# yzhang511/multi_modal_foundation_model

Measured on AMD Instinct MI355X. Metric: pretrain samples/sec (T=100 bins/modality, d_model=256, 5+5 layers, spike+behaviour masked pretraining step), higher is better.
Workload: dtype bf16; 1 GPU; BASELINE.json configs[1]: 1 session, ap(668 neurons)+behaviour(2), d_model=256, heads=8, mlp=512, 5 enc + 5 dec layers, T=100 (L=200 tokens), dropout 0.4/0.2, AdamW+OneCycleLR, mixed objectives; per_gpu_batch=1024, global_batch=1024, seq_len=200, parallelism=dp1

## Files before the change

include/mmfm.h:

```cpp
#ifndef MMFM_H
#define MMFM_H
#include <stdint.h>
#ifdef __cplusplus
extern "C" {
#endif

#define MMFM_VERSION 401
#define MMFM_F32 0
#define MMFM_BF16 1
#define MMFM_MLP_GELU 0
#define MMFM_MLP_RELU 1
#define MMFM_MLP_SIGMOID 2
#define MMFM_MLP_GELU_TANH 3

typedef void* mmfm_stream;

typedef struct {
    const void* state;
    uint32_t site;
    float p;
} mmfm_dropout;

int mmfm_version(void);
const char* mmfm_last_error(void);
// ... 134 lines not shown
    float* bp;
    int N, K;
    int tile0;
    int scalar_gain;
    void* WpP;
    void* WpTP;
} mmfm_prep_entry;
int mmfm_prep_weights(const mmfm_prep_entry* entries, int n_entries, int total_tiles, mmfm_stream stream);

typedef struct {
    int64_t R;
    int K, N;
    const void* x; int ldx;
    const void* w; int ldw;
    const float* bias;
    int ln; float eps;
    void* xhat; float* rstd;
    const void* residual; int ldr;
    void* y; int ldy;
    int stream_out;
    int rotate;
    int ln_bwd;
    const void* bwd_xhat; const float* bwd_rstd;
} mmfm_rowgemm_desc;
int mmfm_rowgemm(const mmfm_rowgemm_desc* d, mmfm_stream stream);

typedef struct {
    int64_t R;
    const void* x; int ldx;
    float eps;
    const void* w_up; const float* b_up;
    const void* w_down; const float* b_down;
    mmfm_dropout drop;
    void* y; int ldy;
    void* xhat; float* rstd;
    const void* dy; int lddy;
    const void* w_down_t;
    const void* w_up_t;
    void* t1; void* g; void* du;
    void* dx; int lddx;
    int rotate;
    int scalenorm;
    int act;
    float act_beta;
} mmfm_mlp_desc;
int mmfm_mlp_fwd(const mmfm_mlp_desc* d, mmfm_stream stream);
// ... 14 lines not shown
```

multi_modal_foundation_model_amd/_lib.py:

```python
from __future__ import annotations

import ctypes as C
import os
import re

import torch

_HERE = os.path.dirname(os.path.abspath(__file__))
LIB_PATH = os.environ.get("MMFM_LIB") or os.path.join(_HERE, "libmmfm_hip.so")
HEADER_PATH = os.path.join(os.path.dirname(_HERE), "include", "mmfm.h")

F32, BF16 = 0, 1
ATTN_DIAG, ATTN_CAUSAL, ATTN_SEP = 1, 2, 4
ACT_NONE, ACT_GELU, ACT_SOFTSIGN, ACT_GELU_GRAD, ACT_SOFTSIGN_GRAD, ACT_SOFTSIGN_GRAD_OUT = 0, 1, 2, 3, 4, 5
ACT_RELU, ACT_RELU_GRAD, ACT_SIGMOID, ACT_SIGMOID_GRAD, ACT_GELU_TANH, ACT_GELU_TANH_GRAD = 6, 7, 8, 9, 10, 11
MLP_GELU, MLP_RELU, MLP_SIGMOID, MLP_GELU_TANH = 0, 1, 2, 3


class MmfmError(RuntimeError):
    pass


class Dropout(C.Structure):
    _fields_ = [("state", C.c_void_p), ("site", C.c_uint32), ("p", C.c_float)]
# ... 15 lines not shown
    _fields_ = [("dtype", C.c_int), ("B", C.c_int), ("heads", C.c_int), ("Lq", C.c_int), ("Lk", C.c_int), ("dh", C.c_int),
                ("q", C.c_void_p), ("k", C.c_void_p), ("v", C.c_void_p), ("ldq", C.c_int), ("ldk", C.c_int),
                ("ldv", C.c_int), ("o", C.c_void_p), ("ldo", C.c_int), ("lse", C.c_void_p), ("keypad", C.c_void_p),
                ("mod_id", C.c_void_p), ("flags", C.c_int), ("scale", C.c_float), ("drop_p", Dropout),
                ("drop_o", Dropout), ("d_o", C.c_void_p), ("lddo", C.c_int), ("dq", C.c_void_p), ("dk", C.c_void_p),
                ("dv", C.c_void_p), ("lddq", C.c_int), ("lddk", C.c_int), ("lddv", C.c_int), ("keepbits", C.c_void_p)]


class PrepEntry(C.Structure):
    _fields_ = [("W", C.c_void_p), ("gamma", C.c_void_p), ("beta", C.c_void_p), ("bias", C.c_void_p), ("Wp", C.c_void_p),
                ("WpT", C.c_void_p), ("bp", C.c_void_p), ("N", C.c_int), ("K", C.c_int), ("tile0", C.c_int), ("scalar_gain", C.c_int),
                ("WpP", C.c_void_p), ("WpTP", C.c_void_p)]


class ReduceEntry(C.Structure):
    _fields_ = [("dst", C.c_void_p), ("src", C.c_void_p), ("n", C.c_int64), ("slab_stride", C.c_int64), ("nslabs", C.c_int32),
                ("accumulate", C.c_int32), ("chunk0", C.c_int32), ("pad_", C.c_int32)]


class RowGemmDesc(C.Structure):
    _fields_ = [("R", C.c_int64), ("K", C.c_int), ("N", C.c_int), ("x", C.c_void_p), ("ldx", C.c_int), ("w", C.c_void_p),
                ("ldw", C.c_int), ("bias", C.c_void_p), ("ln", C.c_int), ("eps", C.c_float), ("xhat", C.c_void_p),
                ("rstd", C.c_void_p), ("residual", C.c_void_p), ("ldr", C.c_int), ("y", C.c_void_p), ("ldy", C.c_int),
                ("stream_out", C.c_int), ("rotate", C.c_int), ("ln_bwd", C.c_int), ("bwd_xhat", C.c_void_p), ("bwd_rstd", C.c_void_p)]


class MlpDesc(C.Structure):
    _fields_ = [("R", C.c_int64), ("x", C.c_void_p), ("ldx", C.c_int), ("eps", C.c_float), ("w_up", C.c_void_p),
                ("b_up", C.c_void_p), ("w_down", C.c_void_p), ("b_down", C.c_void_p), ("drop", Dropout), ("y", C.c_void_p),
                ("ldy", C.c_int), ("xhat", C.c_void_p), ("rstd", C.c_void_p), ("dy", C.c_void_p), ("lddy", C.c_int),
                ("w_down_t", C.c_void_p), ("w_up_t", C.c_void_p), ("t1", C.c_void_p), ("g", C.c_void_p), ("du", C.c_void_p),
                ("dx", C.c_void_p), ("lddx", C.c_int), ("rotate", C.c_int), ("scalenorm", C.c_int),
                ("act", C.c_int), ("act_beta", C.c_float)]


_vp, _i, _i64, _f = C.c_void_p, C.c_int, C.c_int64, C.c_float
_PROTOS = {
    "mmfm_version": (C.c_int, []),
    "mmfm_last_error": (C.c_char_p, []),
    "mmfm_device_check": (C.c_int, [_i]),
    "mmfm_rng_seed": (C.c_int, [_vp, C.c_uint64, _vp]),
    "mmfm_rng_advance": (C.c_int, [_vp, _vp]),
    "mmfm_gemm": (C.c_int, [C.POINTER(GemmDesc), _vp]),
    "mmfm_gemm_pair": (C.c_int, [_vp, _vp, _vp]),
    "mmfm_gemm_dw_tiles": (C.c_int, [_i, _i, _i]),
    "mmfm_reduce_slabs": (C.c_int, [_vp, _vp, _i64, _i, _i64, _i, _vp]),
    "mmfm_reduce_slabs_multi": (C.c_int, [_vp, _i, _i, _vp]),
# ... 66 lines not shown
```

multi_modal_foundation_model_amd/csrc/rowgemm.hip:

```cpp
#define MMFM_ACT_LOAD_AUX 2
#include "rowchain.h"
#include <stdlib.h>
#include <algorithm>
#include <type_traits>

using namespace rowchain;

namespace {

constexpr int NT = 256, NW = 4;

constexpr int BIAS_MAX = 1024;

template <int KP, int LN, bool NTS, int NWV>
__global__ __launch_bounds__(NWV * 64, (KP == 1 ? 2 : 1)) void rowgemm_kernel(const mmfm_rowgemm_desc d) {
    constexpr int NT = NWV * 64, NW = NWV;
    __shared__ __attribute__((aligned(16))) char smem[LDS_BYTES + NW * STG_BYTES + BIAS_MAX * 4];
    const int t = threadIdx.x, lane = t & 63, wave = __builtin_amdgcn_readfirstlane(t >> 6), m = lane & 31, h = lane >> 5;
    const int npair = d.N >> 6, cpp = 2 * npair * KP;
    const int64_t npass = (d.R + 32 * NW - 1) / (32 * NW);
    const int my_passes = blockIdx.x < npass ? (int)((npass - 1 - blockIdx.x) / gridDim.x) + 1 : 0;
    if (my_passes == 0) return;
    const uint16_t* W = reinterpret_cast<const uint16_t*>(d.w);
    const int ldw = d.ldw;
// ... 218 lines not shown
            f32x16 o[2];
#pragma unroll
            for (int j = 0; j < 2; ++j) {
                const f32x16 xt = unstage_tile(xstash + tp * STG_BYTES, j, m, h);
#pragma unroll
                for (int i = 0; i < 16; ++i) o[j][i] = rs * (acc[2 * tp + j][i] - s1 - xt[i] * s2);
            }
            stage_lines(stg, rl, lane);
#pragma unroll
            for (int j = 0; j < 2; ++j) {
                const f32x16 r = unstage_tile(stg, j, m, h);
#pragma unroll
                for (int i = 0; i < 16; ++i) o[j][i] += r[i];
            }
            stage_tile(stg, 0, m, h, o[0]);
            stage_tile(stg, 1, m, h, o[1]);
            flush_lines<false>(stg, Y, wrow0, ldyb, 128u * tp, lane);
        }
    }
}

#pragma clang diagnostic push
#pragma clang diagnostic ignored "-Winline-asm"
template <int KP, int NORM>
__global__ __launch_bounds__(NT) void rowgemm_lnbwd_a_kernel(const mmfm_rowgemm_desc d) {
    constexpr int RING_B = RINGA_SLOTS * CHUNK;
    extern __shared__ __attribute__((aligned(16))) char smem[];
    const int t = threadIdx.x, lane = t & 63, wave = __builtin_amdgcn_readfirstlane(t >> 6), m = lane & 31, h = lane >> 5;
    constexpr int cpp = 8 * KP;
    const int64_t npass = (d.R + 32 * NW - 1) / (32 * NW);
    const int my_passes = blockIdx.x < npass ? (int)((npass - 1 - blockIdx.x) / gridDim.x) + 1 : 0;
    if (my_passes == 0) return;
    const __amdgpu_buffer_rsrc_t rs_w = wbuf(d.w);
    const uint32_t ldwb = (uint32_t)d.ldw * 2u;
    auto src = [=](int g) {
        const int idx = g % cpp, tt = idx / KP, p = idx - tt * KP;
        AChunk c;
        c.rs = rs_w; c.off = (uint32_t)(32 * tt) * ldwb + 512u * (uint32_t)p; c.ldb = ldwb; c.kind = 0;
        return c;
    };
    char* stg = smem + RING_B + wave * STG_BYTES;
    char* xstash = smem + RING_B + NW * STG_BYTES + wave * 4 * STG_BYTES;
    const GBuf X = gbuf(d.x, d.R * d.ldx * 2), Y = gbuf(d.y, d.R * d.ldy * 2), RES = gbuf(d.residual, d.R * d.ldr * 2);
    const GBuf XH = gbuf(d.bwd_xhat, d.R * 512), RS = gbuf(d.bwd_rstd, d.R * 4);
    const uint32_t ldxb = d.ldx * 2, ldyb = d.ldy * 2, ldrb = d.ldr * 2;
    const ALane<NT> ring_al = alane_init<NT>(t, ldwb, 0u);
    const AFrag fr = afrag_init(m, h);
    RINGA_DECL(NT);
    RINGA_START((uint32_t)(uintptr_t)(__attribute__((address_space(3))) char*)smem, my_passes * cpp, src);
    for (int pi = 0; pi < my_passes; ++pi) {
        const uint32_t wrow0 = (uint32_t)(((int64_t)(blockIdx.x + (int64_t)pi * gridDim.x) * NW + wave) * 32);
        opnd x[16 * KP];
        {
            Lines xl[4];
#pragma unroll
            for (int tp = 0; tp < 4; ++tp) xl[tp] = fetch_lines(XH, wrow0, 512u, 128u * tp, lane);
            load_rows_lines<4 * KP>(stg, x, X, wrow0, ldxb, lane, m, h);
#pragma unroll
            for (int tp = 0; tp < 4; ++tp) stage_lines(xstash + tp * STG_BYTES, xl[tp], lane);
        }
        float rs = ld4f(RS, (wrow0 + m) * 4u);
        f32x16 acc[8];
#pragma unroll
        for (int tt = 0; tt < 8; ++tt) {
            acc[tt] = zero16();
#pragma unroll
            for (int p = 0; p < KP; ++p) {
                uint32_t slot;
                RINGA_SYNC(src, slot, 0);
                acc[tt] = mma16a<4>(slot, fr, x + 16 * p, acc[tt], [&](int g_) { RINGA_PIECE(g_); });
            }
        }
        float s1 = 0.f, s2 = 0.f;
#pragma unroll
        for (int tp = 0; tp < 4; ++tp) {
#pragma unroll
            for (int j = 0; j < 2; ++j) {
                const f32x16 xt = unstage_tile(xstash + tp * STG_BYTES, j, m, h);
#pragma unroll
                for (int i = 0; i < 16; ++i) { s1 += acc[2 * tp + j][i]; s2 = fmaf(acc[2 * tp + j][i], xt[i], s2); }
            }
        }
        s1 = xhalf(s1);
        s2 = xhalf(s2);
        norm_bwd_stats<NORM>(s1, s2, rs);
        Lines rl4[4];
#pragma unroll
        for (int tp = 0; tp < 4; ++tp) rl4[tp] = fetch_lines(RES, wrow0, ldrb, 128u * tp, lane);
#pragma unroll
        for (int tp = 0; tp < 4; ++tp) {
            const Lines& rl = rl4[tp];
            f32x16 o[2];
#pragma unroll
            for (int j = 0; j < 2; ++j) {
                const f32x16 xt = unstage_tile(xstash + tp * STG_BYTES, j, m, h);
#pragma unroll
                for (int i = 0; i < 16; ++i) o[j][i] = rs * (acc[2 * tp + j][i] - s1 - xt[i] * s2);
            }
            stage_lines(stg, rl, lane);
#pragma unroll
            for (int j = 0; j < 2; ++j) {
                const f32x16 r = unstage_tile(stg, j, m, h);
#pragma unroll
                for (int i = 0; i < 16; ++i) o[j][i] += r[i];
            }
            stage_tile(stg, 0, m, h, o[0]);
            stage_tile(stg, 1, m, h, o[1]);
            flush_lines<false>(stg, Y, wrow0, ldyb, 128u * tp, lane);
        }
    }
}
#pragma clang diagnostic pop

template <int KP, int NORM>
__global__ __launch_bounds__(512) void rowgemm_lnbwd8_kernel(const mmfm_rowgemm_desc d) {
    constexpr int NT = 512, NW = 8, NPAIR = 4;
    __shared__ __attribute__((aligned(16))) char smem[2 * CHUNK2 + NW * STG_BYTES + NW * 32 * 8];
    const int t = threadIdx.x, lane = t & 63, wave = __builtin_amdgcn_readfirstlane(t >> 6), m = lane & 31, h = lane >> 5;
    const int half = wave >> 2, pw = wave & 3;
    constexpr int cpp = 4 * KP;
    const int64_t npass = (d.R + 32 * NPAIR - 1) / (32 * NPAIR);
    const int my_passes = blockIdx.x < npass ? (int)((npass - 1 - blockIdx.x) / gridDim.x) + 1 : 0;
    if (my_passes == 0) return;
    const uint16_t* W = reinterpret_cast<const uint16_t*>(d.w);
    const int ldw = d.ldw;
    auto src = [=](int g) {
        const int idx = g % cpp, p = idx >> 2, j = idx & 3;
        WChunk2 c;
        c.s[0].base = W + (size_t)(32 * j) * ldw + 256 * p; c.s[0].ld = ldw; c.s[0].kind = 0;
        c.s[1].base = W + (size_t)(32 * (4 + j)) * ldw + 256 * p; c.s[1].ld = ldw; c.s[1].kind = 0;
        return c;
    };
    char* stg = smem + 2 * CHUNK2 + wave * STG_BYTES;
// ... 126 lines not shown
    return (int)std::max<int64_t>(1, std::min<int64_t>(npass, 256 * per_cu));
}

}

extern "C" int mmfm_rowgemm(const mmfm_rowgemm_desc* dp, mmfm_stream stream) {
    const mmfm_rowgemm_desc d = *dp;
    MMFM_REQUIRE(d.x && d.w && d.y && d.R > 0, "mmfm_rowgemm: null operand / empty problem");
    MMFM_REQUIRE(d.K == 256 || d.K == 512 || d.K == 768, "mmfm_rowgemm: K = %d (256, 512 or 768 only)", d.K);
    MMFM_REQUIRE(d.N > 0 && d.N % 64 == 0, "mmfm_rowgemm: N = %d must be a positive multiple of 64", d.N);
    MMFM_REQUIRE(d.ldx % 8 == 0 && d.ldw % 8 == 0 && d.ldy % 8 == 0 && d.ldx >= d.K && d.ldw >= d.K && d.ldy >= d.N,
                 "mmfm_rowgemm: leading dimensions (%d, %d, %d) must be multiples of 8 and cover the rows", d.ldx, d.ldw, d.ldy);
    auto al16 = [](const void* p) { return ((uintptr_t)p & 15) == 0; };
    MMFM_REQUIRE(al16(d.x) && al16(d.w) && al16(d.y) && al16(d.residual) && al16(d.xhat) && al16(d.bwd_xhat) && al16(d.bias),
                 "mmfm_rowgemm: operands must be 16-byte aligned");
    MMFM_REQUIRE(!d.residual || (d.ldr % 8 == 0 && d.ldr >= d.N), "mmfm_rowgemm: ldr %d", d.ldr);
    MMFM_REQUIRE(d.ln >= 0 && d.ln <= 2 && d.ln_bwd >= 0 && d.ln_bwd <= 2, "mmfm_rowgemm: ln = %d, ln_bwd = %d (0, 1 = LayerNorm, 2 = ScaleNorm)", d.ln, d.ln_bwd);
    MMFM_REQUIRE(!d.ln || d.K == 256, "mmfm_rowgemm: the norm prologue needs K = 256");
    const int64_t maxld = std::max<int64_t>(std::max(d.ldx, d.ldy), std::max(d.ldr, 256));
    MMFM_REQUIRE((d.R + 128) * maxld * 2 < (int64_t)1 << 31, "mmfm_rowgemm: tensors beyond 2 GiB are not addressable by the 32-bit buffer offsets");
    MMFM_REQUIRE(d.N <= BIAS_MAX, "mmfm_rowgemm: N = %d > %d", d.N, BIAS_MAX);
    static const int per_cu_env = [] { const char* e = getenv("MMFM_ROWGEMM_WG_PER_CU"); return e ? atoi(e) : 0; }();
    hipStream_t st = (hipStream_t)stream;
    if (d.ln_bwd) {
        MMFM_REQUIRE(d.N == 256 && d.bwd_xhat && d.bwd_rstd && !d.ln && !d.bias, "mmfm_rowgemm: ln_bwd needs N = 256, x_hat, rstd, no bias/ln");
        const bool sn = d.ln_bwd == 2;
        if (d.K == 256) {
            dim3 grid(grid_for(d.R, per_cu_env > 0 ? per_cu_env : 1, 4)), block(512);
            if (sn) hipLaunchKernelGGL((rowgemm_lnbwd8_kernel<1, 2>), grid, block, 0, st, d);
            else hipLaunchKernelGGL((rowgemm_lnbwd8_kernel<1, 1>), grid, block, 0, st, d);
        } else {
            dim3 grid(grid_for(d.R, per_cu_env > 0 ? per_cu_env : 1)), block(NT);
            static const int ring_env = [] { const char* e = getenv("MMFM_ROWGEMM_RING"); return (e ? atoi(e) : 3) & 2; }();
            constexpr int LDS_L = RINGA_SLOTS * CHUNK + NW * STG_BYTES + NW * 4 * STG_BYTES;
#define LNB_A(KP, NORM)                                                                                                     \
            {                                                                                                               \
                if (int rc = mmfm_lds_opt_in(reinterpret_cast<const void*>(rowgemm_lnbwd_a_kernel<KP, NORM>), LDS_L, "mmfm_rowgemm")) return rc; \
                hipLaunchKernelGGL((rowgemm_lnbwd_a_kernel<KP, NORM>), grid, block, LDS_L, st, d);                           \
            }
            if (ring_env && d.K == 512) { if (sn) LNB_A(2, 2) else LNB_A(2, 1) }
            else if (ring_env) { if (sn) LNB_A(3, 2) else LNB_A(3, 1) }
            else if (d.K == 512) { if (sn) hipLaunchKernelGGL((rowgemm_lnbwd_kernel<2, 2>), grid, block, 0, st, d); else hipLaunchKernelGGL((rowgemm_lnbwd_kernel<2, 1>), grid, block, 0, st, d); }
            else { if (sn) hipLaunchKernelGGL((rowgemm_lnbwd_kernel<3, 2>), grid, block, 0, st, d); else hipLaunchKernelGGL((rowgemm_lnbwd_kernel<3, 1>), grid, block, 0, st, d); }
#undef LNB_A
        }
    } else {
#define RG_LAUNCH(KP, LN)                                                                                   \
    if (d.stream_out) hipLaunchKernelGGL((rowgemm_kernel<KP, LN, true, 4>), grid, block, 0, st, d);         \
    else hipLaunchKernelGGL((rowgemm_kernel<KP, LN, false, 4>), grid, block, 0, st, d);
        if (d.K != 256) {
            dim3 grid(grid_for(d.R, per_cu_env > 0 ? per_cu_env : 1, 4)), block(256);
            if (d.K == 512) { RG_LAUNCH(2, 0) } else { RG_LAUNCH(3, 0) }
        } else {
            dim3 grid(grid_for(d.R, per_cu_env > 0 ? per_cu_env : 2, 4)), block(256);
            static const int ring_env = [] { const char* e = getenv("MMFM_ROWGEMM_RING"); return (e ? atoi(e) : 3) & 1; }();
            if (ring_env && (!d.residual || (d.N == 256 && !d.ln))) {
                constexpr int LDS_A = RINGA_SLOTS * CHUNK + 4 * STG_BYTES + BIAS_MAX * 4;
#define RGA_LAUNCH(LN, NTS, NPV)                                                                                            \
                {                                                                                                          \
                    if (int rc = mmfm_lds_opt_in(reinterpret_cast<const void*>(rowgemm_a_kernel<LN, NTS, NPV>), LDS_A, "mmfm_rowgemm")) return rc; \
                    hipLaunchKernelGGL((rowgemm_a_kernel<LN, NTS, NPV>), grid, block, LDS_A, st, d);                        \
                }
#define RGA_LAUNCH2(LN, NPV) if (d.stream_out) RGA_LAUNCH(LN, true, NPV) else RGA_LAUNCH(LN, false, NPV)
                const int64_t npass = (d.R + 127) / 128;
                const int np_all = d.N >> 6;
                static const int nsplit_env = [] { const char* e = getenv("MMFM_ROWGEMM_NSPLIT"); return e ? atoi(e) : 1; }();
// ... 26 lines not shown
```

multi_modal_foundation_model_amd/engine.py:

```python
from __future__ import annotations

import math
import os
from dataclasses import dataclass, field
from typing import Dict, List, Optional, Tuple

import torch

from . import _lib as L
from . import ops as K

LOSS_KIND = {"ap": 0, "behavior": 1}
BLOCK_NORMS = ("ln1", "ln2", "query_norm", "context_norm")


@dataclass
class EngineConfig:
    hidden: int
    heads: int
    inter: int
    n_enc: int
    n_dec: int
    max_F: int
    mult: int
# ... 549 lines not shown
                K.gemm_pair(da, db_, plan=plan)
                K.reduce_slabs(self.Gv(a["wname"] + ".weight"), slab2, Na * Ka + Na, Sa, stra, plan=plan)
                K.reduce_slabs(gdb, slab, N * H + N, Sb, strb, plan=plan)
            elif S == 1:
                K.gemm(dYt, xh, gdb, N, H, R, lda=N, ldb=H, ldc=H, a_kcontig=0, b_kcontig=0, dtype=code, c_f32=1,
                       colsum=gdb.data_ptr() + 4 * N * H, plan=plan)
            elif batch_red:
                stride = _align(N * H + N)
                sl = slab_region(S, stride)
                g_site = buf(f"ws/gdb/{len(late_lng)}", (gdb.numel(),), f32)
                K.gemm(dYt, xh, sl, N, H, R, lda=N, ldb=H, ldc=H, a_kcontig=0, b_kcontig=0, splits=S, kchunk=kchunk,
                       slab_stride=stride, dtype=code, c_f32=1, colsum=sl.data_ptr() + 4 * N * H, plan=plan)
                pend.append((g_site, sl, N * H + N, S, stride, False))
                late_lng.append((g_site, wname, lnname, N))
                return
            else:
                stride = _align(N * H + N)
                slab_fits(slab, S, stride, wname)
                K.gemm(dYt, xh, slab, N, H, R, lda=N, ldb=H, ldc=H, a_kcontig=0, b_kcontig=0, splits=S, kchunk=kchunk,
                       slab_stride=stride, dtype=code, c_f32=1, colsum=slab.data_ptr() + 4 * N * H, plan=plan)
                K.reduce_slabs(gdb, slab, N * H + N, S, stride, plan=plan)
            lin_norm_grad(plan, gdb, wname, lnname, N)

        def dx_ln(plan, dYt, Kd, tag, wname, lnname, dres, dXout):
            K.rowgemm(dYt, prep["v"][wname]["WpT"], dXout, R, H, Kd, ldw=Kd, residual=dres, ldr=H if dres is not None else 0,
                      ln_bwd=2 if self.is_sn(lnname) else 1, bwd_xhat=self.b[tag + "/xh"], bwd_rstd=self.b[tag + "/rs"], plan=plan)

        enc_flags = L.ATTN_DIAG
        dec_flags = (L.ATTN_CAUSAL if c.causal_mask else 0) | (L.ATTN_SEP if c.sep_mask else 0)

        K.mask_prep(B, T, [self.b[f"mask/{m}"] for m in range(M)], [1] * M, attn, [n for _, n in c.mods], tokmask, keypad, keep0,
                    mod_id, count, plan=fwd)
        tok_tmp = buf("tok_tmp", (BT, H))
        x_enc, emb_enc, x_dec = buf("x_enc", (R, H)), buf("emb_enc", (R, H)), buf("x_dec", (R, H))
        for side, xs, es_ in (("encoder", x_enc, emb_enc), ("decoder", x_dec, None)):
            for m, (mod, n) in enumerate(c.mods):
                p = f"{side}_embeddings.{mod}.embedder"
                n2 = n * c.mult
                a = buf(f"{side}/a/{m}", (BT, n2))
                z = None if code == L.BF16 else buf(f"{side}/z/{m}", (BT, n2))
                lin(fwd, self.b[f"in/{m}"], p + ".token_embed", a, BT, n2, n, ldx=_align(n, 8), pre_out=z, act=L.ACT_SOFTSIGN, act_scale=c.embed_scale)
                lin(fwd, a, p + ".projection", tok_tmp, BT, H, n2, drop=self._drop(f"{side}/embdrop/{m}", dpe))
                mod_row = self.Pf(f"encoder_embeddings.{mod}.embedder.mod_emb.weight")[m]
                K.stitch_fwd(tok_tmp, mod_row, self.Pf(p + ".pos_embed.weight"), ts, keep0, xs, es_, B, T, Lq, m, H, c.max_F, plan=fwd)

        def out_proj(plan, a, wname, Xres, Xout):
            if F_OUT:
                K.rowgemm(a, self.W(wname + ".weight"), Xout, R, H, H, bias=self.Pf(wname + ".bias"), residual=Xres, ldr=H, plan=plan)
            else:
# ... 82 lines not shown
            nonlocal cur
            if pend:
                K.reduce_slabs_multi(list(pend), self.device, plan=cur)
                pend.clear()
            for g_site, wname, lnname, N in late_lng:
                lin_norm_grad(cur, g_site, wname, lnname, N)
            late_lng.clear()
            slabm_off[0] = 0
            bwd.append((name, cur))
            cur = []

        dY = buf("d/stream", (R, H))
        dydec = buf("d/ydec", (R, H))
        t1, t2, dh_ = buf("d/t1", (R, H)), buf("d/t2", (R, H)), buf("d/h", (R, H))
        du, dqkv, dctx = buf("d/u", (R, I)), buf("d/qkv", (R, 3 * H)), buf("d/ctx", (R, H))
        for m, (mod, n) in enumerate(c.mods):
            dpred = buf(f"d/pred/{m}", (BT, n))
            K.masked_loss_bwd(c.loss_kind[mod], self.b[f"pred/{m}"], self.b[f"tgt/{m}"], tokmask[:, m * T:], Lq, T, BT, n,
                              self.b["gout"], self.b["inv_n"], dpred, plan=cur)
            dlin(cur, dpred, ydec[m * BT:(m + 1) * BT], f"decoder_embeddings.{mod}.out", BT, n, H, dX=dydec[m * BT:(m + 1) * BT])
        ln_b(cur, dydec, dec_last, "decoder_norm", "decnorm", None, dY, ds_L=Lq, ds_T=T)
        close_segment("head")

        def mlp_back(plan, dS, p, tag, X_in):
            if F_MLP:
                pu, pdn = prep["v"][p + ".mlp.up_proj"], prep["v"][p + ".mlp.down_proj"]
                t1b, gb, dub = buf("d/t1m", (R, H)), buf("d/g", (R, I)), buf("d/du", (R, I))
                split = os.environ.get("MMFM_MLP_BWD_SPLIT", "1") == "1" or self.is_sn(p + ".ln2")
                d_ = K.mlp_desc(R, w_up=pu["Wp"], b_up=pu["bp"], drop=self._drop(tag + "/mlpdrop", dp), xhat=self.b[tag + "/ln2/xh"],
                                rstd=self.b[tag + "/ln2/rs"], dy=dS, w_down_t=pdn["WpT"], w_up_t=pu["WpTP"], t1=t1b, g=gb, du=dub,
                                dx=None if split else dS, act=c.act[0], act_beta=c.act[1])
                K.mlp_bwd(d_, plan=plan)
                if split:
                    dx_ln(plan, dub, I, tag + "/ln2", p + ".mlp.up_proj", p + ".ln2", dS, dS)
                dlin(plan, t1b, gb, p + ".mlp.down_proj", R, H, I, defer=True)
                dlin_ln(plan, dub, tag + "/ln2", p + ".mlp.up_proj", p + ".ln2", I)
                flush_deferred(plan)
                return
            dSd = dS
            if dp > 0:
                K.dropout_apply(dS, t1, R, H, self._drop(tag + "/mlpdrop", dp), plan=plan)
                dSd = t1
            dlin(plan, dSd, self.b[tag + "/g"], p + ".mlp.down_proj", R, H, I, dX=du, act=act_grad, act_scale=c.act[1],
                 gradmul_pre=self.b[tag + "/u"])
            dlin(plan, du, self.b[tag + "/h2"], p + ".mlp.up_proj", R, I, H, dX=dh_)
            ln_b(plan, dh_, X_in, p + ".ln2", tag + "/ln2", dS, dS)

        def out_proj_back(plan, dS, a, wname):
            if F_OUT:
                dlin(plan, dS, a, wname, R, H, H, defer=True)
                K.rowgemm(dS, prep["v"][wname]["WpT"], t2, R, H, H, plan=plan)
            else:
                dlin(plan, dS, a, wname, R, H, H, dX=t2)

        def self_back(plan, dS, p, tag, X_in, flags):
            out_proj_back(plan, dS, self.b[tag + "/a"], p + ".attn.out_proj")
            qkv = self.b[tag + "/qkv"]
            K.attn_bwd(attn_desc(tag + "/sa", qkv, 3 * H, qkv, 3 * H, H, 2 * H, self.b[tag + "/a"], flags, d_o=t2, dq=dqkv, dkv=dqkv,
                                 lddq=3 * H, lddkv=3 * H, dkoff=H, dvoff=2 * H), plan=plan)
            if F_QKV:
                dlin_ln(plan, dqkv, tag + "/ln1", p + ".attn.qkv", p + ".ln1", 3 * H)
                flush_deferred(plan)
                dx_ln(plan, dqkv, 3 * H, tag + "/ln1", p + ".attn.qkv", p + ".ln1", dS, dS)
            else:
                flush_deferred(plan)
                dlin(plan, dqkv, self.b[tag + "/h1"], p + ".attn.qkv", R, 3 * H, H, dX=dh_)
                ln_b(plan, dh_, X_in, p + ".ln1", tag + "/ln1", dS, dS)

        dqc, dkvc = buf("d/qc", (R, H)), buf("d/kvc", (R, 2 * H))
        first_ctx = True
        for i in reversed(range(c.n_dec)):
            p, tag = f"decoder.{i}", f"dec{i}"
            mlp_back(cur, dY, p, tag, self.b[tag + "/yb"])
            out_proj_back(cur, dY, self.b[tag + "/a2"], p + ".cross_attn.out_proj")
            K.attn_bwd(attn_desc(tag + "/xa", self.b[tag + "/qc"], H, self.b[tag + "/kvc"], 2 * H, 0, H, self.b[tag + "/a2"], enc_flags,
                                 d_o=t2, dq=dqc, dkv=dkvc, lddq=H, lddkv=2 * H, dkoff=0, dvoff=H), plan=cur)
            if F_LNL:
                dlin_ln(cur, dqc, tag + "/qn", p + ".cross_attn.query", p + ".query_norm", H)
                flush_deferred(cur)
                dx_ln(cur, dqc, H, tag + "/qn", p + ".cross_attn.query", p + ".query_norm", dY, dY)
                dlin_ln(cur, dkvc, tag + "/cn", p + ".cross_attn.kv", p + ".context_norm", 2 * H)
                dx_ln(cur, dkvc, 2 * H, tag + "/cn", p + ".cross_attn.kv", p + ".context_norm", None if first_ctx else dctx, dctx)
            else:
                flush_deferred(cur)
                dlin(cur, dqc, self.b[tag + "/hq"], p + ".cross_attn.query", R, H, H, dX=dh_)
                ln_b(cur, dh_, self.b[tag + "/xa"], p + ".query_norm", tag + "/qn", dY, dY)
                dlin(cur, dkvc, self.b[tag + "/hc"], p + ".cross_attn.kv", R, 2 * H, H, dX=dh_)
                ln_b(cur, dh_, context, p + ".context_norm", tag + "/cn", None if first_ctx else dctx, dctx)
            first_ctx = False
            self_back(cur, dY, p, tag, stream_in[tag], dec_flags)
            close_segment(p)
        if c.n_dec == 0:
            raise NotImplementedError("n_dec == 0")
        dX = buf("d/xstream", (R, H))
        if F_LNL:
            dlin_ln(cur, dctx, "encnorm", "decoder_proj_context", "encoder_norm", H)
            dx_ln(cur, dctx, H, "encnorm", "decoder_proj_context", "encoder_norm", None, dX)
        else:
            dlin(cur, dctx, enc_out, "decoder_proj_context", R, H, H, dX=dh_)
            ln_b(cur, dh_, enc_last, "encoder_norm", "encnorm", None, dX)
        close_segment("bridge")
        for i in reversed(range(c.n_enc)):
            p, tag = f"encoder.{i}", f"enc{i}"
            mlp_back(cur, dX, p, tag, self.b[tag + "/xa"])
            self_back(cur, dX, p, tag, stream_in[tag], enc_flags)
            close_segment(p)
        for side, dS, dextra, acc_mod in (("decoder", dY, None, False), ("encoder", dX, dctx, True)):
            for m, (mod, n) in enumerate(c.mods):
                pS = f"{side}_embeddings.{mod}.embedder"
                K.stitch_bwd(dS, dextra, ts, keep0, self._drop(f"{side}/embdrop/{m}", dpe), buf(f"d/tok/{side}/{m}", (BT, H)),
                             self.Gv(f"encoder_embeddings.{mod}.embedder.mod_emb.weight")[m], self.Gv(pS + ".pos_embed.weight"),
                             acc_mod, False, B, T, Lq, m, H, c.max_F, ws_st, plan=cur)
        for side in ("decoder", "encoder"):
            for m, (mod, n) in enumerate(c.mods):
                p = f"{side}_embeddings.{mod}.embedder"
                n2 = n * c.mult
                dz = buf(f"d/z/{m}", (BT, n2))
                if code == L.BF16:
                    dlin(cur, self.b[f"d/tok/{side}/{m}"], self.b[f"{side}/a/{m}"], p + ".projection", BT, H, n2, dX=dz,
                         act=L.ACT_SOFTSIGN_GRAD_OUT, act_scale=c.embed_scale, gradmul_pre=self.b[f"{side}/a/{m}"])
                else:
                    dlin(cur, self.b[f"d/tok/{side}/{m}"], self.b[f"{side}/a/{m}"], p + ".projection", BT, H, n2, dX=dz,
                         act=L.ACT_SOFTSIGN_GRAD, act_scale=c.embed_scale, gradmul_pre=self.b[f"{side}/z/{m}"])
                dlin(cur, dz, self.b[f"in/{m}"], p + ".token_embed", BT, n2, n, ldx=_align(n, 8))
        close_segment("embed")
        if used_wt:
            tw = self._wt_table()
            K.prep_weights(tw["table"], tw["n"], tw["tiles"], plan=fwd)
# ... 96 lines not shown
```

multi_modal_foundation_model_amd/ops.py:

```python
from __future__ import annotations

import ctypes as C

import torch

from . import _lib as L


def _stream():
    return torch.cuda.current_stream().cuda_stream


def run_plan(plan, stream=None):
    st = _stream() if stream is None else stream
    for fn, args, _keep in plan:
        rc = fn(*args, st)
        if rc:
            L.check(rc, fn.__name__)


def _emit(plan, fn, args, keep=()):
    if plan is None:
        L.check(fn(*args, _stream()), fn.__name__)
    else:
# ... 181 lines not shown
            raise ValueError(f"prep_table: entry {i}: WpP (unit-permuted along K) needs K % 16 == 0, got K = {Kd} (include/mmfm.h)")
        if e.get("WpTP") is not None and N % 16:
            raise ValueError(f"prep_table: entry {i}: WpTP (unit-permuted along N) needs N % 16 == 0, got N = {N} (include/mmfm.h)")
        a = arr[i]
        a.W, a.gamma, a.beta, a.bias = P(e["W"]), P(e.get("gamma")), P(e.get("beta")), P(e.get("bias"))
        a.Wp, a.WpT, a.bp = P(e.get("Wp")), P(e.get("WpT")), P(e.get("bp"))
        a.WpP, a.WpTP = P(e.get("WpP")), P(e.get("WpTP"))
        if e.get("scalar_gain"):
            if e.get("gamma") is None or e["gamma"].numel() != 1 or e.get("beta") is not None:
                raise ValueError(f"prep_table: entry {i}: scalar_gain needs a one-element gamma and no beta")
            a.scalar_gain = 1
        a.N, a.K, a.tile0 = N, Kd, tile0
        tile0 += (N + 31) // 32
    raw = np.frombuffer(bytes(arr), dtype=np.uint8).copy()
    table = torch.from_numpy(raw).to(device)
    return table, len(entries), tile0


def prep_weights(table, n, tiles, plan=None):
    _emit(plan, L.lib().mmfm_prep_weights, (P(table), n, tiles), keep=(table,))


def rowgemm(x, w, y, R, N, K, *, ldx=None, ldw=None, ldy=None, bias=None, ln=False, eps=1e-5, xhat=None, rstd=None, residual=None,
            ldr=0, stream_out=False, ln_bwd=False, bwd_xhat=None, bwd_rstd=None, rotate=True, plan=None):
    d = L.RowGemmDesc()
    d.R, d.K, d.N = R, K, N
    d.x, d.ldx, d.w, d.ldw = P(x), K if ldx is None else ldx, P(w), K if ldw is None else ldw
    d.bias, d.ln, d.eps, d.xhat, d.rstd = P(bias), int(ln), eps, P(xhat), P(rstd)
    d.residual, d.ldr, d.y, d.ldy = P(residual), ldr, P(y), N if ldy is None else ldy
    d.stream_out, d.ln_bwd, d.bwd_xhat, d.bwd_rstd, d.rotate = int(stream_out), int(ln_bwd), P(bwd_xhat), P(bwd_rstd), int(rotate)
    _emit(plan, L.lib().mmfm_rowgemm, (C.byref(d),), keep=(d,))


MLP_ACTS = {
    "gelu": (L.MLP_GELU, 1.0),
    "relu": (L.MLP_RELU, 1.0),
    "silu": (L.MLP_SIGMOID, 1.0), "swish": (L.MLP_SIGMOID, 1.0), "quick_gelu": (L.MLP_SIGMOID, 1.702),
    "gelu_new": (L.MLP_GELU_TANH, 1.0), "gelu_pytorch_tanh": (L.MLP_GELU_TANH, 1.0), "gelu_fast": (L.MLP_GELU_TANH, 1.0),
}
GEMM_ACTS = {L.MLP_GELU: (L.ACT_GELU, L.ACT_GELU_GRAD), L.MLP_RELU: (L.ACT_RELU, L.ACT_RELU_GRAD),
             L.MLP_SIGMOID: (L.ACT_SIGMOID, L.ACT_SIGMOID_GRAD), L.MLP_GELU_TANH: (L.ACT_GELU_TANH, L.ACT_GELU_TANH_GRAD)}


def mlp_act(name):
    if name not in MLP_ACTS:
        raise NotImplementedError(f"MLP act {name!r} has no kernel; accepted: {', '.join(MLP_ACTS)}")
    return MLP_ACTS[name]


def mlp_desc(R, *, x=None, ldx=256, eps=1e-5, w_up=None, b_up=None, w_down=None, b_down=None, drop=None, y=None, ldy=256, xhat=None,
             rstd=None, dy=None, lddy=256, w_down_t=None, w_up_t=None, t1=None, g=None, du=None, dx=None, lddx=256, rotate=True,
             scalenorm=False, act=L.MLP_GELU, act_beta=1.0):
    d = L.MlpDesc()
# ... 31 lines not shown
```

Baseline: 35650 samples/s.

## Chain out_proj backward GEMM into layernorm-backward rowgemm kernel

Extends the ring-buffered layernorm-backward rowgemm kernel with an optional chained second GEMM. The freshly computed dX tile stays in registers and is multiplied by the next layer's out_proj transposed weight, writing t2 directly. The engine enables this by default for the mlp/query-norm backward and skips the separate out_proj dX rowgemm. This removes one kernel launch and a re-read of dS per layer, at the cost of more register and LDS pressure plus a new K=256 path that replaces the specialised lnbwd8 kernel when chaining.

```diff
diff --git a/include/mmfm.h b/include/mmfm.h
--- a/include/mmfm.h
+++ b/include/mmfm.h
@@ -180,6 +180,8 @@
     int rotate;
     int ln_bwd;
     const void* bwd_xhat; const float* bwd_rstd;
+    const void* chain_w; int ldcw;
+    void* chain_y; int ldcy;
 } mmfm_rowgemm_desc;
 int mmfm_rowgemm(const mmfm_rowgemm_desc* d, mmfm_stream stream);
 
diff --git a/multi_modal_foundation_model_amd/_lib.py b/multi_modal_foundation_model_amd/_lib.py
--- a/multi_modal_foundation_model_amd/_lib.py
+++ b/multi_modal_foundation_model_amd/_lib.py
@@ -61,7 +61,8 @@
     _fields_ = [("R", C.c_int64), ("K", C.c_int), ("N", C.c_int), ("x", C.c_void_p), ("ldx", C.c_int), ("w", C.c_void_p),
                 ("ldw", C.c_int), ("bias", C.c_void_p), ("ln", C.c_int), ("eps", C.c_float), ("xhat", C.c_void_p),
                 ("rstd", C.c_void_p), ("residual", C.c_void_p), ("ldr", C.c_int), ("y", C.c_void_p), ("ldy", C.c_int),
-                ("stream_out", C.c_int), ("rotate", C.c_int), ("ln_bwd", C.c_int), ("bwd_xhat", C.c_void_p), ("bwd_rstd", C.c_void_p)]
+                ("stream_out", C.c_int), ("rotate", C.c_int), ("ln_bwd", C.c_int), ("bwd_xhat", C.c_void_p), ("bwd_rstd", C.c_void_p),
+                ("chain_w", C.c_void_p), ("ldcw", C.c_int), ("chain_y", C.c_void_p), ("ldcy", C.c_int)]
 
 
 class MlpDesc(C.Structure):
diff --git a/multi_modal_foundation_model_amd/csrc/rowgemm.hip b/multi_modal_foundation_model_amd/csrc/rowgemm.hip
--- a/multi_modal_foundation_model_amd/csrc/rowgemm.hip
+++ b/multi_modal_foundation_model_amd/csrc/rowgemm.hip
@@ -264,21 +264,24 @@
 
 #pragma clang diagnostic push
 #pragma clang diagnostic ignored "-Winline-asm"
-template <int KP, int NORM>
+template <int KP, int NORM, bool CHAIN>
 __global__ __launch_bounds__(NT) void rowgemm_lnbwd_a_kernel(const mmfm_rowgemm_desc d) {
     constexpr int RING_B = RINGA_SLOTS * CHUNK;
     extern __shared__ __attribute__((aligned(16))) char smem[];
     const int t = threadIdx.x, lane = t & 63, wave = __builtin_amdgcn_readfirstlane(t >> 6), m = lane & 31, h = lane >> 5;
-    constexpr int cpp = 8 * KP;
+    constexpr int cpm = 8 * KP, cpp = cpm + (CHAIN ? 8 : 0);
     const int64_t npass = (d.R + 32 * NW - 1) / (32 * NW);
     const int my_passes = blockIdx.x < npass ? (int)((npass - 1 - blockIdx.x) / gridDim.x) + 1 : 0;
     if (my_passes == 0) return;
-    const __amdgpu_buffer_rsrc_t rs_w = wbuf(d.w);
-    const uint32_t ldwb = (uint32_t)d.ldw * 2u;
+    const __amdgpu_buffer_rsrc_t rs_w = wbuf(d.w), rs_cw = wbuf(CHAIN ? d.chain_w : d.w);
+    const uint32_t ldwb = (uint32_t)d.ldw * 2u, ldcwb = CHAIN ? (uint32_t)d.ldcw * 2u : ldwb;
+    auto is_chain = [=](int g) { return CHAIN && g % cpp >= cpm; };
     auto src = [=](int g) {
         const int idx = g % cpp, tt = idx / KP, p = idx - tt * KP;
         AChunk c;
-        c.rs = rs_w; c.off = (uint32_t)(32 * tt) * ldwb + 512u * (uint32_t)p; c.ldb = ldwb; c.kind = 0;
+        c.kind = 0;
+        if (CHAIN && idx >= cpm) { c.rs = rs_cw; c.off = (uint32_t)(32 * (idx - cpm)) * ldcwb; c.ldb = ldcwb; }
+        else { c.rs = rs_w; c.off = (uint32_t)(32 * tt) * ldwb + 512u * (uint32_t)p; c.ldb = ldwb; }
         return c;
     };
     char* stg = smem + RING_B + wave * STG_BYTES;
@@ -286,10 +289,16 @@
     const GBuf X = gbuf(d.x, d.R * d.ldx * 2), Y = gbuf(d.y, d.R * d.ldy * 2), RES = gbuf(d.residual, d.R * d.ldr * 2);
     const GBuf XH = gbuf(d.bwd_xhat, d.R * 512), RS = gbuf(d.bwd_rstd, d.R * 4);
     const uint32_t ldxb = d.ldx * 2, ldyb = d.ldy * 2, ldrb = d.ldr * 2;
-    const ALane<NT> ring_al = alane_init<NT>(t, ldwb, 0u);
+    const GBuf CY = gbuf(CHAIN ? d.chain_y : nullptr, d.R * d.ldcy * 2);
+    const uint32_t ldcyb = d.ldcy * 2;
+    const ALane<NT> ring_al = alane_init<NT>(t, ldwb, 0u), chain_al = alane_init<NT>(t, ldcwb, 0u);
     const AFrag fr = afrag_init(m, h);
     RINGA_DECL(NT);
     RINGA_START((uint32_t)(uintptr_t)(__attribute__((address_space(3))) char*)smem, my_passes * cpp, src);
+#define LNB_LANE()                                                                                           \
+        ALane<NT> al_n = ring_al;                                                                            \
+        if (CHAIN && is_chain(min(ring_cc + 1, ring_last))) al_n = chain_al
+#define LNB_PIECE(Q) dma_piece<NT>(ring_nd, ring_nc, al_n, wave, (Q))
     for (int pi = 0; pi < my_passes; ++pi) {
         const uint32_t wrow0 = (uint32_t)(((int64_t)(blockIdx.x + (int64_t)pi * gridDim.x) * NW + wave) * 32);
         opnd x[16 * KP];
@@ -310,47 +319,98 @@
             for (int p = 0; p < KP; ++p) {
                 uint32_t slot;
                 RINGA_SYNC(src, slot, 0);
-                acc[tt] = mma16a<4>(slot, fr, x + 16 * p, acc[tt], [&](int g_) { RINGA_PIECE(g_); });
+                LNB_LANE();
+                acc[tt] = mma16a<4>(slot, fr, x + 16 * p, acc[tt], [&](int g_) { LNB_PIECE(g_); });
             }
         }
         float s1 = 0.f, s2 = 0.f;
-#pragma unroll
-        for (int tp = 0; tp < 4; ++tp) {
-#pragma unroll
-            for (int j = 0; j < 2; ++j) {
-                const f32x16 xt = unstage_tile(xstash + tp * STG_BYTES, j, m, h);
-#pragma unroll
-                for (int i = 0; i < 16; ++i) { s1 += acc[2 * tp + j][i]; s2 = fmaf(acc[2 * tp + j][i], xt[i], s2); }
-            }
-        }
-        s1 = xhalf(s1);
-        s2 = xhalf(s2);
+        if constexpr (KP == 1) {
+            float sa[2] = {0.f, 0.f}, sb[2] = {0.f, 0.f};
+#pragma unroll
+            for (int tp = 0; tp < 4; ++tp) {
+#pragma unroll
+                for (int j = 0; j < 2; ++j) {
+                    const f32x16 xt = unstage_tile(xstash + tp * STG_BYTES, j, m, h);
+#pragma unroll
+                    for (int i = 0; i < 16; ++i) { sa[tp >> 1] += acc[2 * tp + j][i]; sb[tp >> 1] = fmaf(acc[2 * tp + j][i], xt[i], sb[tp >> 1]); }
+                }
+            }
+            s1 = xhalf(sa[0]) + xhalf(sa[1]);
+            s2 = xhalf(sb[0]) + xhalf(sb[1]);
+        } else {
+#pragma unroll
+            for (int tp = 0; tp < 4; ++tp) {
+#pragma unroll
+                for (int j = 0; j < 2; ++j) {
+                    const f32x16 xt = unstage_tile(xstash + tp * STG_BYTES, j, m, h);
+#pragma unroll
+                    for (int i = 0; i < 16; ++i) { s1 += acc[2 * tp + j][i]; s2 = fmaf(acc[2 * tp + j][i], xt[i], s2); }
+                }
+            }
+            s1 = xhalf(s1);
+            s2 = xhalf(s2);
+        }
         norm_bwd_stats<NORM>(s1, s2, rs);
         Lines rl4[4];
 #pragma unroll
         for (int tp = 0; tp < 4; ++tp) rl4[tp] = fetch_lines(RES, wrow0, ldrb, 128u * tp, lane);
+        opnd cx[CHAIN ? 16 : 1];
 #pragma unroll
         for (int tp = 0; tp < 4; ++tp) {
             const Lines& rl = rl4[tp];
             f32x16 o[2];
-#pragma unroll
-            for (int j = 0; j < 2; ++j) {
-                const f32x16 xt = unstage_tile(xstash + tp * STG_BYTES, j, m, h);
-#pragma unroll
-                for (int i = 0; i < 16; ++i) o[j][i] = rs * (acc[2 * tp + j][i] - s1 - xt[i] * s2);
-            }
-            stage_lines(stg, rl, lane);
-#pragma unroll
-            for (int j = 0; j < 2; ++j) {
-                const f32x16 r = unstage_tile(stg, j, m, h);
-#pragma unroll
-                for (int i = 0; i < 16; ++i) o[j][i] += r[i];
+            if constexpr (KP == 1) {
+                stage_lines(stg, rl, lane);
+#pragma unroll
+                for (int j = 0; j < 2; ++j) {
+                    const f32x16 xt = unstage_tile(xstash + tp * STG_BYTES, j, m, h);
+                    const f32x16 r = unstage_tile(stg, j, m, h);
+#pragma unroll
+                    for (int i = 0; i < 16; ++i) o[j][i] = r[i] + rs * (acc[2 * tp + j][i] - s1 - xt[i] * s2);
+                }
+            } else {
+#pragma unroll
+                for (int j = 0; j < 2; ++j) {
+                    const f32x16 xt = unstage_tile(xstash + tp * STG_BYTES, j, m, h);
+#pragma unroll
+                    for (int i = 0; i < 16; ++i) o[j][i] = rs * (acc[2 * tp + j][i] - s1 - xt[i] * s2);
+                }
+                stage_lines(stg, rl, lane);
+#pragma unroll
+                for (int j = 0; j < 2; ++j) {
+                    const f32x16 r = unstage_tile(stg, j, m, h);
+#pragma unroll
+                    for (int i = 0; i < 16; ++i) o[j][i] += r[i];
+                }
             }
             stage_tile(stg, 0, m, h, o[0]);
             stage_tile(stg, 1, m, h, o[1]);
+            if constexpr (CHAIN) {
+#pragma unroll
+                for (int s = 0; s < 4; ++s) cx[4 * tp + s] = unstage_opnd(stg, s, m, h);
+            }
             flush_lines<false>(stg, Y, wrow0, ldyb, 128u * tp, lane);
         }
-    }
+        if constexpr (CHAIN) {
+#pragma unroll
+            for (int tp = 0; tp < 4; ++tp) {
+                f32x16 c2[2];
+#pragma unroll
+                for (int j = 0; j < 2; ++j) {
+                    uint32_t slot;
+                    if (tp == 0) vm_wait_n<1024 / NT + 16>(); else vm_wait_n<1024 / NT + 4>();
+                    RINGA_SYNC_NOWAIT(src, slot);
+                    LNB_LANE();
+                    c2[j] = mma16a<4>(slot, fr, cx, zero16(), [&](int g_) { LNB_PIECE(g_); });
+                }
+                stage_tile(stg, 0, m, h, c2[0]);
+                stage_tile(stg, 1, m, h, c2[1]);
+                flush_lines<false>(stg, CY, wrow0, ldcyb, 128u * tp, lane);
+            }
+        }
+    }
+#undef LNB_PIECE
+#undef LNB_LANE
 }
 #pragma clang diagnostic pop
 
@@ -523,10 +583,17 @@
     MMFM_REQUIRE(d.N <= BIAS_MAX, "mmfm_rowgemm: N = %d > %d", d.N, BIAS_MAX);
     static const int per_cu_env = [] { const char* e = getenv("MMFM_ROWGEMM_WG_PER_CU"); return e ? atoi(e) : 0; }();
     hipStream_t st = (hipStream_t)stream;
+    const bool chain = d.chain_w != nullptr || d.chain_y != nullptr;
+    if (chain) {
+        MMFM_REQUIRE(d.chain_w && d.chain_y && al16(d.chain_w) && al16(d.chain_y), "mmfm_rowgemm: chain_w and chain_y go together, 16-byte aligned");
+        MMFM_REQUIRE(d.ldcw % 8 == 0 && d.ldcw >= 256 && d.ldcy % 8 == 0 && d.ldcy >= 256, "mmfm_rowgemm: chain leading dimensions (%d, %d)", d.ldcw, d.ldcy);
+        MMFM_REQUIRE((d.R + 128) * (int64_t)d.ldcy * 2 < (int64_t)1 << 31, "mmfm_rowgemm: chain_y beyond 2 GiB is not addressable by the 32-bit buffer offsets");
+        if (!d.ln_bwd) return -1000;
+    }
     if (d.ln_bwd) {
         MMFM_REQUIRE(d.N == 256 && d.bwd_xhat && d.bwd_rstd && !d.ln && !d.bias, "mmfm_rowgemm: ln_bwd needs N = 256, x_hat, rstd, no bias/ln");
         const bool sn = d.ln_bwd == 2;
-        if (d.K == 256) {
+        if (d.K == 256 && !chain) {
             dim3 grid(grid_for(d.R, per_cu_env > 0 ? per_cu_env : 1, 4)), block(512);
             if (sn) hipLaunchKernelGGL((rowgemm_lnbwd8_kernel<1, 2>), grid, block, 0, st, d);
             else hipLaunchKernelGGL((rowgemm_lnbwd8_kernel<1, 1>), grid, block, 0, st, d);
@@ -534,15 +601,19 @@
             dim3 grid(grid_for(d.R, per_cu_env > 0 ? per_cu_env : 1)), block(NT);
             static const int ring_env = [] { const char* e = getenv("MMFM_ROWGEMM_RING"); return (e ? atoi(e) : 3) & 2; }();
             constexpr int LDS_L = RINGA_SLOTS * CHUNK + NW * STG_BYTES + NW * 4 * STG_BYTES;
-#define LNB_A(KP, NORM)                                                                                                     \
+#define LNB_A(KP, NORM, CH)                                                                                                 \
             {                                                                                                               \
-                if (int rc = mmfm_lds_opt_in(reinterpret_cast<const void*>(rowgemm_lnbwd_a_kernel<KP, NORM>), LDS_L, "mmfm_rowgemm")) return rc; \
-                hipLaunchKernelGGL((rowgemm_lnbwd_a_kernel<KP, NORM>), grid, block, LDS_L, st, d);                           \
-            }
-            if (ring_env && d.K == 512) { if (sn) LNB_A(2, 2) else LNB_A(2, 1) }
-            else if (ring_env) { if (sn) LNB_A(3, 2) else LNB_A(3, 1) }
+                if (int rc = mmfm_lds_opt_in(reinterpret_cast<const void*>(rowgemm_lnbwd_a_kernel<KP, NORM, CH>), LDS_L, "mmfm_rowgemm")) return rc; \
+                hipLaunchKernelGGL((rowgemm_lnbwd_a_kernel<KP, NORM, CH>), grid, block, LDS_L, st, d);                       \
+            }
+#define LNB_A2(KP, NORM) if (chain) LNB_A(KP, NORM, true) else LNB_A(KP, NORM, false)
+            if (chain && !ring_env) return -1000;
+            if (chain && d.K == 256) { if (sn) LNB_A(1, 2, true) else LNB_A(1, 1, true) }
+            else if (ring_env && d.K == 512) { if (sn) LNB_A2(2, 2) else LNB_A2(2, 1) }
+            else if (ring_env) { if (sn) LNB_A2(3, 2) else LNB_A2(3, 1) }
             else if (d.K == 512) { if (sn) hipLaunchKernelGGL((rowgemm_lnbwd_kernel<2, 2>), grid, block, 0, st, d); else hipLaunchKernelGGL((rowgemm_lnbwd_kernel<2, 1>), grid, block, 0, st, d); }
             else { if (sn) hipLaunchKernelGGL((rowgemm_lnbwd_kernel<3, 2>), grid, block, 0, st, d); else hipLaunchKernelGGL((rowgemm_lnbwd_kernel<3, 1>), grid, block, 0, st, d); }
+#undef LNB_A2
 #undef LNB_A
         }
     } else {
diff --git a/multi_modal_foundation_model_amd/engine.py b/multi_modal_foundation_model_amd/engine.py
--- a/multi_modal_foundation_model_amd/engine.py
+++ b/multi_modal_foundation_model_amd/engine.py
@@ -595,9 +595,14 @@
                 K.reduce_slabs(gdb, slab, N * H + N, S, stride, plan=plan)
             lin_norm_grad(plan, gdb, wname, lnname, N)
 
-        def dx_ln(plan, dYt, Kd, tag, wname, lnname, dres, dXout):
+        chain_bwd = (bool(fm) and F_OUT and bool(int(os.environ.get("MMFM_ROWCHAIN", "3")) & 1)
+                     and bool(int(os.environ.get("MMFM_ROWGEMM_RING", "3")) & 2) and (R + 127) // 128 >= 128)
+
+        def dx_ln(plan, dYt, Kd, tag, wname, lnname, dres, dXout, chain=None):
             K.rowgemm(dYt, prep["v"][wname]["WpT"], dXout, R, H, Kd, ldw=Kd, residual=dres, ldr=H if dres is not None else 0,
-                      ln_bwd=2 if self.is_sn(lnname) else 1, bwd_xhat=self.b[tag + "/xh"], bwd_rstd=self.b[tag + "/rs"], plan=plan)
+                      ln_bwd=2 if self.is_sn(lnname) else 1, bwd_xhat=self.b[tag + "/xh"], bwd_rstd=self.b[tag + "/rs"],
+                      chain_w=None if chain is None else prep["v"][chain]["WpT"], chain_y=None if chain is None else self.b["d/t2"],
+                      plan=plan)
 
         enc_flags = L.ATTN_DIAG
         dec_flags = (L.ATTN_CAUSAL if c.causal_mask else 0) | (L.ATTN_SEP if c.sep_mask else 0)
@@ -726,7 +731,7 @@
         ln_b(cur, dydec, dec_last, "decoder_norm", "decnorm", None, dY, ds_L=Lq, ds_T=T)
         close_segment("head")
 
-        def mlp_back(plan, dS, p, tag, X_in):
+        def mlp_back(plan, dS, p, tag, X_in, chain=None):
             if F_MLP:
                 pu, pdn = prep["v"][p + ".mlp.up_proj"], prep["v"][p + ".mlp.down_proj"]
                 t1b, gb, dub = buf("d/t1m", (R, H)), buf("d/g", (R, I)), buf("d/du", (R, I))
@@ -736,11 +741,11 @@
                                 dx=None if split else dS, act=c.act[0], act_beta=c.act[1])
                 K.mlp_bwd(d_, plan=plan)
                 if split:
-                    dx_ln(plan, dub, I, tag + "/ln2", p + ".mlp.up_proj", p + ".ln2", dS, dS)
+                    dx_ln(plan, dub, I, tag + "/ln2", p + ".mlp.up_proj", p + ".ln2", dS, dS, chain=chain)
                 dlin(plan, t1b, gb, p + ".mlp.down_proj", R, H, I, defer=True)
                 dlin_ln(plan, dub, tag + "/ln2", p + ".mlp.up_proj", p + ".ln2", I)
                 flush_deferred(plan)
-                return
+                return split and chain is not None
             dSd = dS
             if dp > 0:
                 K.dropout_apply(dS, t1, R, H, self._drop(tag + "/mlpdrop", dp), plan=plan)
@@ -749,16 +754,18 @@
                  gradmul_pre=self.b[tag + "/u"])
             dlin(plan, du, self.b[tag + "/h2"], p + ".mlp.up_proj", R, I, H, dX=dh_)
             ln_b(plan, dh_, X_in, p + ".ln2", tag + "/ln2", dS, dS)
-
-        def out_proj_back(plan, dS, a, wname):
+            return False
+
+        def out_proj_back(plan, dS, a, wname, chained=False):
             if F_OUT:
                 dlin(plan, dS, a, wname, R, H, H, defer=True)
-                K.rowgemm(dS, prep["v"][wname]["WpT"], t2, R, H, H, plan=plan)
+                if not chained:
+                    K.rowgemm(dS, prep["v"][wname]["WpT"], t2, R, H, H, plan=plan)
             else:
                 dlin(plan, dS, a, wname, R, H, H, dX=t2)
 
-        def self_back(plan, dS, p, tag, X_in, flags):
-            out_proj_back(plan, dS, self.b[tag + "/a"], p + ".attn.out_proj")
+        def self_back(plan, dS, p, tag, X_in, flags, chained=False):
+            out_proj_back(plan, dS, self.b[tag + "/a"], p + ".attn.out_proj", chained=chained)
             qkv = self.b[tag + "/qkv"]
             K.attn_bwd(attn_desc(tag + "/sa", qkv, 3 * H, qkv, 3 * H, H, 2 * H, self.b[tag + "/a"], flags, d_o=t2, dq=dqkv, dkv=dqkv,
                                  lddq=3 * H, lddkv=3 * H, dkoff=H, dvoff=2 * H), plan=plan)
@@ -775,14 +782,14 @@
         first_ctx = True
         for i in reversed(range(c.n_dec)):
             p, tag = f"decoder.{i}", f"dec{i}"
-            mlp_back(cur, dY, p, tag, self.b[tag + "/yb"])
-            out_proj_back(cur, dY, self.b[tag + "/a2"], p + ".cross_attn.out_proj")
+            chained = mlp_back(cur, dY, p, tag, self.b[tag + "/yb"], chain=p + ".cross_attn.out_proj" if chain_bwd else None)
+            out_proj_back(cur, dY, self.b[tag + "/a2"], p + ".cross_attn.out_proj", chained=chained)
             K.attn_bwd(attn_desc(tag + "/xa", self.b[tag + "/qc"], H, self.b[tag + "/kvc"], 2 * H, 0, H, self.b[tag + "/a2"], enc_flags,
                                  d_o=t2, dq=dqc, dkv=dkvc, lddq=H, lddkv=2 * H, dkoff=0, dvoff=H), plan=cur)
             if F_LNL:
                 dlin_ln(cur, dqc, tag + "/qn", p + ".cross_attn.query", p + ".query_norm", H)
                 flush_deferred(cur)
-                dx_ln(cur, dqc, H, tag + "/qn", p + ".cross_attn.query", p + ".query_norm", dY, dY)
+                dx_ln(cur, dqc, H, tag + "/qn", p + ".cross_attn.query", p + ".query_norm", dY, dY, chain=p + ".attn.out_proj" if chain_bwd else None)
                 dlin_ln(cur, dkvc, tag + "/cn", p + ".cross_attn.kv", p + ".context_norm", 2 * H)
                 dx_ln(cur, dkvc, 2 * H, tag + "/cn", p + ".cross_attn.kv", p + ".context_norm", None if first_ctx else dctx, dctx)
             else:
@@ -792,7 +799,7 @@
                 dlin(cur, dkvc, self.b[tag + "/hc"], p + ".cross_attn.kv", R, 2 * H, H, dX=dh_)
                 ln_b(cur, dh_, context, p + ".context_norm", tag + "/cn", None if first_ctx else dctx, dctx)
             first_ctx = False
-            self_back(cur, dY, p, tag, stream_in[tag], dec_flags)
+            self_back(cur, dY, p, tag, stream_in[tag], dec_flags, chained=chain_bwd and F_LNL)
             close_segment(p)
         if c.n_dec == 0:
             raise NotImplementedError("n_dec == 0")
@@ -806,8 +813,8 @@
         close_segment("bridge")
         for i in reversed(range(c.n_enc)):
             p, tag = f"encoder.{i}", f"enc{i}"
-            mlp_back(cur, dX, p, tag, self.b[tag + "/xa"])
-            self_back(cur, dX, p, tag, stream_in[tag], enc_flags)
+            chained = mlp_back(cur, dX, p, tag, self.b[tag + "/xa"], chain=p + ".attn.out_proj" if chain_bwd else None)
+            self_back(cur, dX, p, tag, stream_in[tag], enc_flags, chained=chained)
             close_segment(p)
         for side, dS, dextra, acc_mod in (("decoder", dY, None, False), ("encoder", dX, dctx, True)):
             for m, (mod, n) in enumerate(c.mods):
diff --git a/multi_modal_foundation_model_amd/ops.py b/multi_modal_foundation_model_amd/ops.py
--- a/multi_modal_foundation_model_amd/ops.py
+++ b/multi_modal_foundation_model_amd/ops.py
@@ -227,13 +227,16 @@
 
 
 def rowgemm(x, w, y, R, N, K, *, ldx=None, ldw=None, ldy=None, bias=None, ln=False, eps=1e-5, xhat=None, rstd=None, residual=None,
-            ldr=0, stream_out=False, ln_bwd=False, bwd_xhat=None, bwd_rstd=None, rotate=True, plan=None):
+            ldr=0, stream_out=False, ln_bwd=False, bwd_xhat=None, bwd_rstd=None, rotate=True, chain_w=None, chain_y=None, ldcw=256,
+            ldcy=256, plan=None):
     d = L.RowGemmDesc()
     d.R, d.K, d.N = R, K, N
     d.x, d.ldx, d.w, d.ldw = P(x), K if ldx is None else ldx, P(w), K if ldw is None else ldw
     d.bias, d.ln, d.eps, d.xhat, d.rstd = P(bias), int(ln), eps, P(xhat), P(rstd)
     d.residual, d.ldr, d.y, d.ldy = P(residual), ldr, P(y), N if ldy is None else ldy
     d.stream_out, d.ln_bwd, d.bwd_xhat, d.bwd_rstd, d.rotate = int(stream_out), int(ln_bwd), P(bwd_xhat), P(bwd_rstd), int(rotate)
+    if chain_w is not None or chain_y is not None:
+        d.chain_w, d.ldcw, d.chain_y, d.ldcy = P(chain_w), ldcw, P(chain_y), ldcy
     _emit(plan, L.lib().mmfm_rowgemm, (C.byref(d),), keep=(d,))
 
 
```

Result: no change. 35890 samples/s (median of 6 runs) (+0.7%).
